# cartgr/Generating-Fair-Consensus-Statements-with-Social-Choice-on-Token-Level-MDPs

Measured on AMD Instinct MI355X. Metric: agent×candidate scorings/sec + decode steps/sec at 1/2/4/8 MI355X; % HBM roofline, higher is better.
Workload: dtype bf16

## Files before the change

### generating-fair-consensus-statements-with-social-choice-on-token-level-mdps_amd/csrc/attn.hip

```cpp
#include "cs_kernels.cuh"

#include <algorithm>
#include <vector>

namespace {

typedef __bf16 bf16x8 __attribute__((ext_vector_type(8)));
typedef __bf16 bf16x4 __attribute__((ext_vector_type(4)));
typedef float f32x4 __attribute__((ext_vector_type(4)));

constexpr int kAttnThreads = 256;
constexpr int kGroupRows = 64;
constexpr int kKeyBlock = 32;
constexpr int kMaxSplit = 32;
constexpr int kPlanMinBase = 1024;
constexpr int kMergeRows = 8;
constexpr float kLazyRescale = 8.0f;
constexpr int64_t kPlanImbalance = 4;
constexpr int kPlanTargetWgs = 512;
constexpr int kPlanMinItems = 3;

struct AttnParams {
  const __bf16* q;
  const __bf16* kp;
// ... 269 lines not shown

template <int D>
__device__ __forceinline__ void fetch_chunks(const BlockRef& r, u32x4 (&rk)[LdsTile<D>::NCH],
                                             u32x4 (&rv)[LdsTile<D>::NCH]) {
#pragma unroll
  for (int j = 0; j < LdsTile<D>::NCH; ++j) {
    const int c = static_cast<int>(threadIdx.x) + kAttnThreads * j;
    rk[j] = *reinterpret_cast<const u32x4*>(r.k + c * 8);
    rv[j] = *reinterpret_cast<const u32x4*>(r.vt + c * 8);
  }
}

template <int D>
__device__ __forceinline__ void stage_chunks(__bf16* buf, int j, const u32x4 (&rk)[LdsTile<D>::NCH],
                                             const u32x4 (&rv)[LdsTile<D>::NCH]) {
  using LT = LdsTile<D>;
  __bf16* kd = buf + (j & 1) * LT::ELEMS;
  __bf16* vd = kd + LT::KELEMS;
  const int tid = threadIdx.x;
  __bf16* kt = kd + (tid / (D / 8)) * LT::KROW + (tid % (D / 8)) * 8;
  __bf16* vt = vd + (tid >> 2) * LT::VROW + (tid & 3) * 8;
#pragma unroll
  for (int i = 0; i < LT::NCH; ++i) {
    *reinterpret_cast<u32x4*>(kt + i * (kAttnThreads / (D / 8)) * LT::KROW) = rk[i];
    *reinterpret_cast<u32x4*>(vt + i * (kAttnThreads / 4) * LT::VROW) = rv[i];
  }
}

__device__ __forceinline__ bool mine_staged(const TileRows& tr, int j) {
  return tr.active && (j % tr.kw) == tr.ks;
}

template <int D, typename Ref>
__device__ __forceinline__ void attend_staged(const AttnParams& a, const TileRows& tr, const __bf16* buf,
                                              int j, Ref ref, const bf16x8 (&qf)[D / 32],
                                              f32x4 (&o)[D / 16], float& m, float& l) {
  using LT = LdsTile<D>;
  const int col = tr.col, h4 = tr.h4;
  const __bf16* kd = buf + (j & 1) * LT::ELEMS;
  const __bf16* vd = kd + LT::KELEMS;
  KeyBlock<D> f;
#pragma unroll
  for (int ds = 0; ds < D / 32; ++ds) {
    f.k0[ds] = *reinterpret_cast<const bf16x8*>(kd + col * LT::KROW + ds * 32 + 8 * h4);
    f.k1[ds] = *reinterpret_cast<const bf16x8*>(kd + (16 + col) * LT::KROW + ds * 32 + 8 * h4);
  }
#pragma unroll
  for (int dt = 0; dt < D / 16; ++dt) {
    f.vlo[dt] = *reinterpret_cast<const bf16x4*>(vd + (dt * 16 + col) * LT::VROW + 4 * h4);
    f.vhi[dt] = *reinterpret_cast<const bf16x4*>(vd + (dt * 16 + col) * LT::VROW + 16 + 4 * h4);
  }
  attend_block<D>(a, f, ref(j).mask, qf, tr.kmin_pos, h4, o, m, l);
}

#define CS_ATTEND_STAGED(D, a, tr, lds, n_blocks, ref, qf, o, m, l)                         \
  do {                                                                                      \
    using LT_ = LdsTile<D>;                                                                 \
    const int n_ = (n_blocks);                                                              \
    __bf16* buf_ = reinterpret_cast<__bf16*>(lds);                                          \
    u32x4 rk_[LT_::NCH], rv_[LT_::NCH];                                                     \
    if (n_ > 0) {                                                                           \
      fetch_chunks<D>(ref(0), rk_, rv_);                                                    \
      stage_chunks<D>(buf_, 0, rk_, rv_);                                                   \
    }                                                                                       \
    __syncthreads();                                                                        \
    for (int j_ = 0; j_ < n_; ++j_) {                                                       \
      const bool more_ = j_ + 1 < n_;                                                       \
      if (more_) fetch_chunks<D>(ref(j_ + 1), rk_, rv_);                                    \
      if (mine_staged(tr, j_)) attend_staged<D>(a, tr, buf_, j_, ref, qf, o, m, l);   \
      if (more_) stage_chunks<D>(buf_, j_ + 1, rk_, rv_);                                   \
      __syncthreads();                                                                      \
    }                                                                                       \
  } while (0)

template <int D>
__device__ __forceinline__ void combine_waves(const TileRows& tr, char* lds, f32x4 (&o)[D / 16],
                                              float& m, float& l) {
  auto sm = reinterpret_cast<float (*)[16][LdsTile<D>::LDSW]>(lds);
  const int n_qt = tr.n_qt, kw = tr.kw, col = tr.col, h4 = tr.h4;
  l += __shfl_xor(l, 16, 64);
  l += __shfl_xor(l, 32, 64);
  if (kw > 1) {
    if (tr.active && tr.ks > 0) {
      const int sl = tr.w - n_qt;
#pragma unroll
      for (int dt = 0; dt < D / 16; ++dt)
#pragma unroll
        for (int i = 0; i < 4; ++i) sm[sl][col][dt * 16 + 4 * h4 + i] = o[dt][i];
      if (h4 == 0) {
        sm[sl][col][D] = m;
        sm[sl][col][D + 1] = l;
      }
    }
    __syncthreads();
    if (tr.active && tr.ks == 0) {
      float mt = m;
      for (int k = 1; k < kw; ++k) mt = fmaxf(mt, sm[tr.qt + n_qt * k - n_qt][col][D]);
      const float c0 = mt == -INFINITY ? 0.0f : __builtin_amdgcn_exp2f(m - mt);
      l *= c0;
#pragma unroll
      for (int dt = 0; dt < D / 16; ++dt) o[dt] *= c0;
      for (int k = 1; k < kw; ++k) {
        const int sl = tr.qt + n_qt * k - n_qt;
        const float mk = sm[sl][col][D];
        const float ck = mt == -INFINITY ? 0.0f : __builtin_amdgcn_exp2f(mk - mt);
        l = fmaf(sm[sl][col][D + 1], ck, l);
#pragma unroll
        for (int dt = 0; dt < D / 16; ++dt)
#pragma unroll
          for (int i = 0; i < 4; ++i) o[dt][i] = fmaf(sm[sl][col][dt * 16 + 4 * h4 + i], ck, o[dt][i]);
      }
      m = mt;
    }
  }
}

template <int D>
__device__ __forceinline__ void store_out(const AttnParams& a, const TileRows& tr,
                                          const f32x4 (&o)[D / 16], float l) {
  const float inv = l > 0.0f ? 1.0f / l : 0.0f;
  __bf16* orow = a.out + (tr.tok * a.H + tr.head) * D + 4 * tr.h4;
#pragma unroll
  for (int dt = 0; dt < D / 16; ++dt) {
    bf16x4 v;
#pragma unroll
    for (int i = 0; i < 4; ++i) v[i] = static_cast<__bf16>(o[dt][i] * inv);
    *reinterpret_cast<bf16x4*>(orow + dt * 16) = v;
  }
}

template <int D>
__global__ __launch_bounds__(kAttnThreads, D <= 128 ? 2 : 1)
void prefix_attn_lds_kernel(AttnParams a) {
  __shared__ __attribute__((aligned(16))) char lds[LdsTile<D>::kBytes];
  const int bid = logical_block(a.swizzle);
  const TileRows tr = tile_rows(a, bid / a.n_qg, bid % a.n_qg);
  const HistBlocks hs = hist_blocks(a, tr.hb, tr.r0, tr.r0 + tr.nrows - 1);
  const int nbp = (tr.pl + kKeyBlock - 1) / kKeyBlock;

  bf16x8 qf[D / 32];
  load_q<D>(a, tr, qf);
  f32x4 o[D / 16];
#pragma unroll
  for (int dt = 0; dt < D / 16; ++dt) o[dt] = f32x4{0.f, 0.f, 0.f, 0.f};
  float m = -INFINITY, l = 0.0f;

  const KvBase kv = kv_base(a);
  auto ref = [&](int it) {
    return it < nbp ? prefix_block<D>(a, kv, tr, it) : hist_block<D>(a, kv, tr, hs, it - nbp);
  };
  CS_ATTEND_STAGED(D, a, tr, lds, nbp + hs.n, ref, qf, o, m, l);
  combine_waves<D>(tr, lds, o, m, l);
  if (tr.vrow && tr.ks == 0) store_out<D>(a, tr, o, l);
}

#ifdef CS_TRACE_ATTN
constexpr int kAttTraceWgs = 4096;
__device__ unsigned long long g_attn_ts[kAttTraceWgs][8];
#define ATT_T(...) __VA_ARGS__
__device__ __forceinline__ void att_at(int i) {
  if (blockIdx.x < kAttTraceWgs) g_attn_ts[blockIdx.x][i] = wall_clock64();
}
#else
#define ATT_T(...)
#endif

template <int D, bool ROWS = false>
__global__ __launch_bounds__(kAttnThreads, 2)
void prefix_attn_plan_lds_kernel(AttnParams a) {
  using LT = LdsTile<D>;
  constexpr int NDS = D / 32;
  constexpr int NDT = D / 16;
  constexpr int kVImg = kKeyBlock * D * 2;
  static_assert(kAttnThreads / 64 * kVImg <= LT::kBufBytes, "the V images fit the prefix buffers");
  __shared__ __attribute__((aligned(16))) char lds[LT::kBytes];

  ATT_T(if (threadIdx.x == 0) att_at(0);)
  const int4 e = a.plan ? a.plan[blockIdx.x]
                        : int4{static_cast<int>(blockIdx.x) / a.n_qg, static_cast<int>(blockIdx.x) % a.n_qg,
                               1 << 8, 0};
  const int split = e.z & 255, n_used = e.z >> 8, slot = e.w;
  const TileRows tr = tile_rows(a, e.x, e.y);
  const int lane = tr.lane, w = tr.w, kw = tr.kw, ks = tr.ks;
  const int col = tr.col, h4 = tr.h4;
  const bool active = tr.active;

  const int nbp = (tr.pl + kKeyBlock - 1) / kKeyBlock;
  const int npi = nbp > split ? (nbp - split + n_used - 1) / n_used : 0;
  ATT_T(if (threadIdx.x == 0 && npi + tr.hb + tr.po >= 0) att_at(1);)
  const int rt0 = tr.r0 + tr.qt * 16;
  const HistBlocks hs = hist_blocks(a, tr.hb, rt0, min(rt0 + 15, tr.M - 1));
  const int n_hist = hs.n;
  const int nslot = n_used * kw;
  auto hrow_of = [&](int ih) -> int32_t {
    const int64_t sg = static_cast<int64_t>(tr.gi) * a.n_str + hs.b_lo + ih / hs.nbh;
    return a.hrow[sg * a.ldh + (ih % hs.nbh) * kKeyBlock + (lane & 31)];
  };
  int32_t hcur = 0;
  if constexpr (ROWS) {
    if (active && split * kw + ks < n_hist) hcur = hrow_of(split * kw + ks);
  }

  bf16x8 qf[NDS];
  load_q<D>(a, tr, qf);
  f32x4 o[NDT];
#pragma unroll
  for (int dt = 0; dt < NDT; ++dt) o[dt] = f32x4{0.f, 0.f, 0.f, 0.f};
  float m = -INFINITY, l = 0.0f;

  const KvBase kv = kv_base(a);
  auto ref = [&](int j) { return prefix_block<D>(a, kv, tr, split + j * n_used); };
  CS_ATTEND_STAGED(D, a, tr, lds, npi, ref, qf, o, m, l);

  ATT_T(if (threadIdx.x == 0) att_at(2);)
  if constexpr (!ROWS) {
    if (active) {
      for (int ih = split * kw + ks; ih < n_hist; ih += nslot) {
        KeyBlock<D> f;
        const BlockRef r = hist_block<D>(a, kv, tr, hs, ih);
        load_block<D>(f, r, col, h4);
        attend_block<D>(a, f, r.mask, qf, tr.kmin_pos, h4, o, m, l);
      }
    }
  } else {
    unsigned char* vimg = reinterpret_cast<unsigned char*>(lds) + w * kVImg;
    constexpr int CPK = D / 8;
    constexpr int KPI = 64 / CPK;
    const int kq = 4 * h4 + ((lane & 15) >> 2);
    const uint32_t tr_base = static_cast<uint32_t>(kq * 2 * D + 8 * (lane & 3));
    const int s2 = vimg_swz<D>(kq) >> 1;
    const int dkey = lane / CPK, dch = lane % CPK;
    typedef __attribute__((address_space(3))) bf16x4* lds_b4_ptr;
    if (active && split * kw + ks < n_hist) {
#pragma unroll
      for (int i = 0; i < kVImg / 1024; ++i)
        *reinterpret_cast<u32x4*>(vimg + 1024 * i + 16 * lane) = u32x4{0u, 0u, 0u, 0u};
    }
    if (active) {
      for (int ih = split * kw + ks; ih < n_hist; ih += nslot) {
        const BlockMask mk = hist_block<D>(a, kv, tr, hs, ih).mask;
        const int kb = mk.kb;
        const int nvalid = min(kKeyBlock, hs.hlim - kb);
        const int n_instr = (nvalid + KPI - 1) / KPI;
        auto row_ptr = [&](const __bf16* base, int64_t srow, int key) {
          return base + ((srow * a.Hkv + tr.g) * a.ldh + kb + key) * D;
        };
        const int64_t rk0 = __shfl(hcur, col, 64), rk1 = __shfl(hcur, 16 + col, 64);
        KeyBlock<D> f;
        const __bf16* kp0 = row_ptr(a.kh, rk0, col) + 8 * h4;
        const __bf16* kp1 = row_ptr(a.kh, rk1, 16 + col) + 8 * h4;
#pragma unroll
        for (int ds = 0; ds < NDS; ++ds) {
          f.k0[ds] = *reinterpret_cast<const bf16x8*>(kp0 + ds * 32);
          f.k1[ds] = *reinterpret_cast<const bf16x8*>(kp1 + ds * 32);
        }
        __builtin_amdgcn_sched_barrier(0);
        asm volatile("s_waitcnt lgkmcnt(0)" ::: "memory");
#pragma unroll 1
        for (int i = 0; i < n_instr; ++i) {
          const int k = i * KPI + dkey;
          const int64_t rv = __shfl(hcur, k, 64);
          const __bf16* vsrc = row_ptr(a.vth, rv, k) + 8 * (dch ^ vimg_swz<D>(k));
          __builtin_amdgcn_global_load_lds(vsrc, (__attribute__((address_space(3))) void*)(vimg + 1024 * i),
                                           16, 0, 0);
        }
        __builtin_amdgcn_sched_barrier(0);
        const int ihn = ih + nslot < n_hist ? ih + nslot : ih;
        const int32_t hnext = hrow_of(ihn);
        __builtin_amdgcn_sched_barrier(0);
        asm volatile("s_waitcnt vmcnt(0)" ::: "memory");
#pragma unroll
        for (int dt = 0; dt < NDT; ++dt) {
          const uint32_t o2 = tr_base + 32 * (((dt & 7) ^ s2) + (dt & ~7));
          f.vlo[dt] = __builtin_amdgcn_ds_read_tr16_b64_v4bf16((lds_b4_ptr)(vimg + o2));
          f.vhi[dt] = __builtin_amdgcn_ds_read_tr16_b64_v4bf16((lds_b4_ptr)(vimg + o2 + 32 * D));
        }
        attend_block<D>(a, f, mk, qf, tr.kmin_pos, h4, o, m, l);
        hcur = hnext;
      }
    }
    __syncthreads();
  }
  ATT_T(if (threadIdx.x == 0 && l >= 0.0f) att_at(3);)
  combine_waves<D>(tr, lds, o, m, l);
  if (!tr.vrow || ks != 0) return;
  if (n_used == 1) {
    store_out<D>(a, tr, o, l);
  } else {
    float* pr = a.part + (static_cast<int64_t>(slot) * kGroupRows + tr.qt * 16 + col) * LT::LDSW;
#pragma unroll
    for (int dt = 0; dt < NDT; ++dt)
      *reinterpret_cast<f32x4*>(pr + dt * 16 + 4 * h4) = o[dt];
    if (h4 == 0) {
      pr[D] = m;
      pr[D + 1] = l;
    }
  }
  ATT_T(if (threadIdx.x == 0) { __builtin_amdgcn_s_waitcnt(0); att_at(4); })
}

#undef CS_ATTEND_STAGED

template <int D>
__global__ __launch_bounds__(kAttnThreads) void attn_merge_kernel(AttnParams a) {
  constexpr int LDSW = D + 2;
  constexpr int NC = D / 4;
// ... 255 lines not shown
  for (int32_t gi = 0; gi < n_groups; ++gi) {
    const int32_t p = group_prefix ? group_prefix[gi] : gi;
    if (p < 0 || p >= n_prefix || prefix_len[p] < 0)
      return fail(CS_ERR_INVALID, "cs_prefix_attention_plan: group_prefix / prefix_len out of range");
    const int64_t nbp = (prefix_len[p] + kKeyBlock - 1) / kKeyBlock;
    for (int64_t qg = 0; qg < n_qg; ++qg) {
      const int64_t r0 = qg * kGroupRows;
      const int64_t nrows = std::min<int64_t>(kGroupRows, M - r0);
      const int64_t n_qt = (nrows + 15) / 16;
      const int64_t kw = n_qt == 1 ? 4 : (n_qt == 2 ? 2 : 1);
      int64_t items = 0;
      for (int64_t q = 0; q < n_qt; ++q) {
        const int64_t rt0 = r0 + 16 * q, rt1 = std::min(rt0 + 15, M - 1);
        const int64_t streams = (rt1 / rep) / T - (rt0 / rep) / T + 1;
        items = std::max(items, nbp + streams * nbh_max);
      }
      cl.push_back({gi, static_cast<int32_t>(qg), items, kw, nrows});
    }
  }
  if (base >= kPlanMinBase) {
    int64_t sum = 0, mx = 0;
    for (const Cell& c : cl) {
      sum += c.items;
      mx = std::max(mx, c.items);
    }
    if (mx * static_cast<int64_t>(cl.size()) <= kPlanImbalance * sum) return 0;
  }
  auto splits_of = [](const Cell& c, int64_t q) {
    return std::max<int64_t>(1, std::min<int64_t>(kMaxSplit, (c.items + q * c.kw - 1) / (q * c.kw)));
  };
  int64_t work = 0;
  for (const Cell& c : cl) work += (c.items + c.kw - 1) / c.kw;
  work *= Hkv;
  const int64_t q = std::max<int64_t>(kPlanMinItems, (work + kPlanTargetWgs - 1) / kPlanTargetWgs);
  std::vector<PlanCell> cells;
  cells.reserve(cl.size());
  int64_t na = 0, nm = 0, slots = 0;
  for (const Cell& c : cl) {
    const int64_t s = splits_of(c, q);
    const int64_t per = (c.items + s * c.kw - 1) / (s * c.kw);
    cells.push_back({c.gi, c.qg, static_cast<int32_t>(s), static_cast<int32_t>(per)});
    na += s * Hkv;
    if (s > 1) {
      slots += s * Hkv;
      nm += (c.nrows + kMergeRows - 1) / kMergeRows * Hkv;
    }
  }
  if (nm == 0) return 0;
  if (na + nm > 0x7fffffffLL) return fail(CS_ERR_INVALID, "cs_prefix_attention_plan: plan too large");
  if (n_attn) *n_attn = static_cast<int32_t>(na);
  if (n_merge) *n_merge = static_cast<int32_t>(nm);
  if (workspace_bytes) *workspace_bytes = static_cast<size_t>(slots) * kGroupRows * (D + 2) * sizeof(float);
  const int64_t total = na + nm;
  if (!plan) return total;
  if (plan_cap < total) return fail(CS_ERR_INVALID, "cs_prefix_attention_plan: plan_cap too small");
  std::stable_sort(cells.begin(), cells.end(),
                   [](const PlanCell& x, const PlanCell& y) { return x.per_wg > y.per_wg; });
  int32_t* pa = plan;
  int32_t* pm = plan + 4 * na;
  int32_t slot = 0;
  for (const PlanCell& c : cells) {
    const int64_t r0 = static_cast<int64_t>(c.qg) * kGroupRows;
    const int64_t nrows = std::min<int64_t>(kGroupRows, M - r0);
    for (int32_t g = 0; g < Hkv; ++g) {
      const int32_t pg = c.gi * Hkv + g;
      for (int32_t sp = 0; sp < c.splits; ++sp) {
        pa[0] = pg;
        pa[1] = c.qg;
        pa[2] = sp | (c.splits << 8);
        pa[3] = c.splits > 1 ? slot + sp : 0;
        pa += 4;
      }
      if (c.splits > 1) {
        for (int32_t ch = 0; ch < (nrows + kMergeRows - 1) / kMergeRows; ++ch) {
          pm[0] = pg;
          pm[1] = c.qg;
          pm[2] = slot;
          pm[3] = ch | (c.splits << 8);
          pm += 4;
        }
        slot += c.splits;
      }
    }
  }
  return total;
}

}

namespace {
int prefix_attention_impl(const char* name, const void* q, const void* k_prefix, const void* vt_prefix,
                          int64_t ld_prefix, const int64_t* prefix_off, const int32_t* prefix_len,
                          int32_t max_prefix_len, const int32_t* group_prefix, int32_t n_groups,
                          const void* k_hist, const void* vt_hist, const int32_t* hist_rows,
                          int64_t ld_hist, const int32_t* hist_base, int32_t n_str, int32_t T,
                          int32_t H, int32_t Hkv, int32_t D, float scale, float softcap,
                          int32_t window, const void* plan, int32_t n_attn, int32_t n_merge,
                          void* out, void* workspace, size_t workspace_bytes, cs_stream_t stream) {
  const std::string nm(name);
  if (n_groups < 0 || n_str < 0 || T < 0) return fail(CS_ERR_INVALID, nm + ": negative size");
  if (n_groups == 0 || n_str == 0 || T == 0) return CS_OK;
  if (Hkv <= 0 || H <= 0 || H % Hkv != 0 || H / Hkv > 64)
    return fail(CS_ERR_INVALID, nm + ": H must be a multiple of Hkv (<= 64 per group)");
  if (D != 64 && D != 128 && D != 256)
    return fail(CS_ERR_INVALID, nm + ": head_dim must be 64, 128 or 256");
  if (ld_prefix <= 0 || ld_prefix % kKeyBlock != 0 || ld_hist <= 0 || ld_hist % kKeyBlock != 0)
    return fail(CS_ERR_INVALID, nm + ": ld_prefix / ld_hist must be positive multiples of 32");
  if (max_prefix_len < 0 || max_prefix_len > ld_prefix)
    return fail(CS_ERR_INVALID, nm + ": max_prefix_len outside [0, ld_prefix]");
  if (!q || !k_prefix || !vt_prefix || !prefix_off || !prefix_len || !k_hist || !vt_hist ||
      !hist_base || !out || (hist_rows == nullptr) != (nm == "cs_prefix_attention"))
    return fail(CS_ERR_INVALID, nm + ": NULL pointer");
  if (!(scale > 0.0f) || softcap < 0.0f) return fail(CS_ERR_INVALID, nm + ": bad scale / softcap");
  if (plan && (n_attn <= 0 || n_merge <= 0))
    return fail(CS_ERR_INVALID, nm + ": a plan needs n_attn > 0 and n_merge > 0");
  if (plan && !workspace)
    return fail(CS_ERR_WORKSPACE, nm + ": a plan needs the workspace cs_prefix_attention_plan() sized");
  const int64_t M = static_cast<int64_t>(n_str) * T * (H / Hkv);
  const int64_t n_qg = (M + kGroupRows - 1) / kGroupRows;
  const int64_t base = static_cast<int64_t>(n_groups) * Hkv * n_qg;
  if (n_qg > 0x7fffffff || base > 0x7fffffffLL) return fail(CS_ERR_INVALID, nm + ": too many query rows");
  AttnParams a;
  a.q = static_cast<const __bf16*>(q);
  a.kp = static_cast<const __bf16*>(k_prefix);
  a.vtp = static_cast<const __bf16*>(vt_prefix);
  a.poff = prefix_off;
  a.plen = prefix_len;
  a.gpfx = group_prefix;
  a.kh = static_cast<const __bf16*>(k_hist);
  a.vth = static_cast<const __bf16*>(vt_hist);
  a.hist_base = hist_base;
  a.hrow = hist_rows;
  a.out = static_cast<__bf16*>(out);
  a.part = static_cast<float*>(workspace);
  a.plan = static_cast<const int4*>(plan);
  a.ldp = ld_prefix;
  a.ldh = ld_hist;
  a.n_grp = n_groups;
  a.n_str = n_str;
  a.T = T;
  a.H = H;
  a.Hkv = Hkv;
  a.rep = H / Hkv;
  a.n_qg = static_cast<int32_t>(n_qg);
  a.n_attn = plan ? n_attn : 0;
  a.scale = scale;
  a.softcap = softcap;
  a.inv_softcap = softcap > 0.0f ? 1.0f / softcap : 0.0f;
  a.window = window > 0 ? window : 0;
  (void)workspace_bytes;
  const int64_t nwg = plan ? n_attn : base;
  a.swizzle = (!plan && nwg % 8 == 0 && nwg >= 64) ? 1 : 0;
  hipStream_t st = static_cast<hipStream_t>(stream);
  const dim3 grid(static_cast<uint32_t>(nwg));
  const dim3 merge_grid(static_cast<uint32_t>(plan ? n_merge : 0));
#define CS_ATTN_LAUNCH(DV)                                                              \
  do {                                                                                  \
    if (hist_rows)                                                                      \
      hipLaunchKernelGGL((prefix_attn_plan_lds_kernel<DV, true>), grid, dim3(kAttnThreads), 0, st, a); \
    else if (plan)                                                                      \
      hipLaunchKernelGGL(prefix_attn_plan_lds_kernel<DV>, grid, dim3(kAttnThreads), 0, st, a); \
    else                                                                                \
      hipLaunchKernelGGL(prefix_attn_lds_kernel<DV>, grid, dim3(kAttnThreads), 0, st, a); \
    if (plan)                                                                           \
      hipLaunchKernelGGL(attn_merge_kernel<DV>, merge_grid, dim3(kAttnThreads), 0, st, a); \
  } while (0)
  if (D == 64) {
    CS_ATTN_LAUNCH(64);
  } else if (D == 128) {
    CS_ATTN_LAUNCH(128);
  } else {
    CS_ATTN_LAUNCH(256);
  }
#undef CS_ATTN_LAUNCH
  return check_launch(name);
}
}

extern "C" {

int cs_prefix_attention(const void* q, const void* k_prefix, const void* vt_prefix,
                        int64_t ld_prefix, const int64_t* prefix_off, const int32_t* prefix_len,
                        int32_t max_prefix_len, const int32_t* group_prefix, int32_t n_groups,
                        const void* k_hist, const void* vt_hist, int64_t ld_hist,
                        const int32_t* hist_base, int32_t n_str, int32_t T, int32_t H, int32_t Hkv,
                        int32_t D, float scale, float softcap, int32_t window, const void* plan,
                        int32_t n_attn, int32_t n_merge, void* out, void* workspace,
                        size_t workspace_bytes, cs_stream_t stream) {
  return prefix_attention_impl("cs_prefix_attention", q, k_prefix, vt_prefix, ld_prefix, prefix_off,
                               prefix_len, max_prefix_len, group_prefix, n_groups, k_hist, vt_hist,
                               nullptr, ld_hist, hist_base, n_str, T, H, Hkv, D, scale, softcap,
                               window, plan, n_attn, n_merge, out, workspace, workspace_bytes, stream);
}

int cs_prefix_attention_rows(const void* q, const void* k_prefix, const void* vt_prefix,
                             int64_t ld_prefix, const int64_t* prefix_off, const int32_t* prefix_len,
                             int32_t max_prefix_len, const int32_t* group_prefix, int32_t n_groups,
                             const void* k_hist, const void* v_hist, const int32_t* hist_rows,
                             int64_t ld_hist, const int32_t* hist_base, int32_t n_str, int32_t T,
                             int32_t H, int32_t Hkv, int32_t D, float scale, float softcap,
                             int32_t window, const void* plan, int32_t n_attn, int32_t n_merge,
                             void* out, void* workspace, size_t workspace_bytes, cs_stream_t stream) {
  if (!hist_rows) return fail(CS_ERR_INVALID, "cs_prefix_attention_rows: NULL hist_rows");
  return prefix_attention_impl("cs_prefix_attention_rows", q, k_prefix, vt_prefix, ld_prefix,
                               prefix_off, prefix_len, max_prefix_len, group_prefix, n_groups,
                               k_hist, v_hist, hist_rows, ld_hist, hist_base, n_str, T, H, Hkv, D,
                               scale, softcap, window, plan, n_attn, n_merge, out, workspace,
                               workspace_bytes, stream);
}

#ifdef CS_TRACE_ATTN
int cs_attn_trace_read(unsigned long long* out) {
  (void)hipMemcpyFromSymbol(out, HIP_SYMBOL(g_attn_ts), sizeof(g_attn_ts));
  static unsigned long long zero[kAttTraceWgs][8];
  (void)hipMemcpyToSymbol(HIP_SYMBOL(g_attn_ts), zero, sizeof(zero));
  return 0;
}
#endif

int cs_hist_rows_update(const int32_t* src_rows, int32_t* dst_rows, const int64_t* parent,
                        const int32_t* hist_base, int64_t S, int32_t ld_hist, int64_t row_base,
                        int64_t n_rows, cs_stream_t stream) {
  if (S < 0 || ld_hist <= 0 || row_base < 0) return fail(CS_ERR_INVALID, "cs_hist_rows_update: bad shape");
  if (row_base + S > n_rows)
    return fail(CS_ERR_INVALID, "cs_hist_rows_update: rows row_base .. row_base + S - 1 exceed the buffer's n_rows");
  if (S == 0) return CS_OK;
  if (!src_rows || !dst_rows || !parent || !hist_base)
    return fail(CS_ERR_INVALID, "cs_hist_rows_update: NULL pointer");
  if (src_rows == dst_rows) return fail(CS_ERR_INVALID, "cs_hist_rows_update: source and destination must differ");
  if (S > 0x7fffffffLL || row_base + S > 0x7fffffffLL || (S * ld_hist + 255) / 256 > 0x7fffffffLL)
    return fail(CS_ERR_INVALID, "cs_hist_rows_update: table too large");
  hipLaunchKernelGGL(hist_rows_kernel, dim3(static_cast<uint32_t>((S * ld_hist + 255) / 256)), dim3(256), 0,
                     static_cast<hipStream_t>(stream), src_rows, dst_rows, parent, hist_base, S, ld_hist,
                     row_base);
  return check_launch("cs_hist_rows_update");
}

}

namespace {
int rope_place_impl(const void* qkv, int64_t ld_qkv, const float* part, int32_t splits,
                    const float* inv_freq, const int32_t* prefix_len, const int32_t* group_prefix,
                    int32_t n_groups, const int32_t* hist_base, int32_t n_str, int32_t T, int32_t H,
                    int32_t Hkv, int32_t D, void* q_out, void* k_hist, void* vt_hist,
                    int64_t ld_hist, int32_t v_rows, cs_stream_t stream) {
  if (n_groups < 0 || n_str < 0 || T < 0) return fail(CS_ERR_INVALID, "cs_rope_place: negative size");
  if (n_groups == 0 || n_str == 0 || T == 0) return CS_OK;
  if (H <= 0 || Hkv <= 0 || D <= 0 || D % 2 != 0 || ld_qkv < static_cast<int64_t>(H + 2 * Hkv) * D)
    return fail(CS_ERR_INVALID, "cs_rope_place: bad head layout");
  if (ld_hist < T) return fail(CS_ERR_INVALID, "cs_rope_place: ld_hist < T");
  if (!inv_freq || !prefix_len || !hist_base || !q_out || !k_hist || !vt_hist)
    return fail(CS_ERR_INVALID, "cs_rope_place: NULL pointer");
  RopeParams r;
  r.qkv = static_cast<const __bf16*>(qkv);
  r.ldqkv = ld_qkv;
  r.part = part;
  r.splits = splits;
  r.inv_freq = inv_freq;
  r.plen = prefix_len;
  r.gpfx = group_prefix;
  r.hist_base = hist_base;
  r.q_out = static_cast<__bf16*>(q_out);
  r.kh = static_cast<__bf16*>(k_hist);
  r.vth = static_cast<__bf16*>(vt_hist);
  r.ldh = ld_hist;
  r.v_rows = v_rows;
  r.n_tok = static_cast<int64_t>(n_groups) * n_str * T;
  r.n_str = n_str;
  r.T = T;
  r.H = H;
  r.Hkv = Hkv;
  r.D = D;
  if (D % 8 != 0 || D > 256) return fail(CS_ERR_INVALID, "cs_rope_place: head_dim must be a multiple of 8, <= 256");
  if (r.n_tok > 0x7fffffffLL) return fail(CS_ERR_INVALID, "cs_rope_place: too many tokens");
  const int64_t n_tiles = ld_hist / 32;
  const int64_t n_vwg = static_cast<int64_t>(n_groups) * n_str * Hkv * n_tiles;
  r.skip_v = (!part && !v_rows && T >= 32 && ld_hist % 32 == 0 && ld_qkv % 8 == 0 &&
              reinterpret_cast<uintptr_t>(qkv) % 16 == 0 && n_vwg <= 0x7fffffffLL) ? 1 : 0;
  const bool p8 = part ? true
                       : (ld_qkv % 8 == 0 && reinterpret_cast<uintptr_t>(qkv) % 16 == 0 && D % 16 == 0);
  const int64_t n_items = static_cast<int64_t>(H + 2 * Hkv) * (D / 2) / (p8 ? 8 : 4);
  const int64_t n_split = (n_items + kRopeItems - 1) / kRopeItems;
  if (r.n_tok * n_split > 0x7fffffffLL) return fail(CS_ERR_INVALID, "cs_rope_place: too many tokens");
  const dim3 grid(static_cast<uint32_t>(r.n_tok * n_split));
  if (part && splits <= 2)
    hipLaunchKernelGGL((rope_place_kernel<8, true, 2>), grid, dim3(256), 0, static_cast<hipStream_t>(stream),
                       r, static_cast<int32_t>(n_split));
  else if (part && splits <= 4)
    hipLaunchKernelGGL((rope_place_kernel<8, true, 4>), grid, dim3(256), 0, static_cast<hipStream_t>(stream),
                       r, static_cast<int32_t>(n_split));
  else if (part)
    hipLaunchKernelGGL((rope_place_kernel<8, true, 8>), grid, dim3(256), 0, static_cast<hipStream_t>(stream),
                       r, static_cast<int32_t>(n_split));
  else if (p8)
    hipLaunchKernelGGL(rope_place_kernel<8>, grid, dim3(256), 0, static_cast<hipStream_t>(stream), r,
                       static_cast<int32_t>(n_split));
  else
    hipLaunchKernelGGL(rope_place_kernel<4>, grid, dim3(256), 0, static_cast<hipStream_t>(stream), r,
                       static_cast<int32_t>(n_split));
  if (r.skip_v)
    hipLaunchKernelGGL(v_tile_place_kernel, dim3(static_cast<uint32_t>(n_vwg)), dim3(256), 0,
                       static_cast<hipStream_t>(stream), r, static_cast<int32_t>(n_tiles));
  return check_launch("cs_rope_place");
}

int rope_place_splitk_impl(const char* name, const float* part, int32_t splits, const float* inv_freq,
// ... 224 lines not shown
```

Baseline: 563.3.

## Add wide 32x32 MFMA attention kernel for unplanned D=128 prefill

Adds a new attention kernel for head dimension 128 that uses 32x32x16 bf16 MFMA tiles, 64-key blocks, register-prefetched double-buffered LDS staging with XOR swizzles, and lazy softmax rescaling. Each wave owns 32 query rows, and the output goes through an LDS image so global stores are coalesced. The kernel is dispatched when no split plan, no history rows, no softcap and no window apply. The aim is higher MFMA throughput and fewer LDS round trips per key block, at the cost of a large, specialised code path with higher register pressure.

Measured after the change: 572.9, median of 6. 1.02x the previous value.

```diff
diff --git a/generating-fair-consensus-statements-with-social-choice-on-token-level-mdps_amd/csrc/attn.hip b/generating-fair-consensus-statements-with-social-choice-on-token-level-mdps_amd/csrc/attn.hip
--- a/generating-fair-consensus-statements-with-social-choice-on-token-level-mdps_amd/csrc/attn.hip
+++ b/generating-fair-consensus-statements-with-social-choice-on-token-level-mdps_amd/csrc/attn.hip
@@ -445,6 +445,329 @@
   CS_ATTEND_STAGED(D, a, tr, lds, nbp + hs.n, ref, qf, o, m, l);
   combine_waves<D>(tr, lds, o, m, l);
   if (tr.vrow && tr.ks == 0) store_out<D>(a, tr, o, l);
+}
+
+typedef float f32x16 __attribute__((ext_vector_type(16)));
+
+constexpr int kWideWaves = 4;
+constexpr int kWideBlock = 64;
+
+template <int D, int NW>
+struct WideLds {
+  static_assert(D == 128, "the chunk swizzles below are written for 256-byte K rows");
+  static constexpr int NT = 64 * NW;
+  static constexpr int KBYTES = kWideBlock * D * 2;
+  static constexpr int VTILE = D * 64;
+  static constexpr int BUF = KBYTES + 2 * VTILE;
+  static constexpr int NCH = kWideBlock * (D / 8) / NT;
+  static constexpr int QIMG = 32 * D * 2;
+  static_assert(NW * QIMG <= 2 * BUF, "every wave's row image fits the two key buffers");
+  static_assert(NCH >= 2 && NCH % 2 == 0, "a thread's chunks split evenly over the two tiles");
+};
+
+template <int NW>
+__device__ __forceinline__ TileRows wide_rows(const AttnParams& a, int pg, int qg) {
+  TileRows r;
+  r.gi = pg / a.Hkv;
+  r.g = pg % a.Hkv;
+  const int p = a.gpfx ? a.gpfx[r.gi] : r.gi;
+  r.M = a.n_str * a.T * a.rep;
+  r.r0 = qg * 32 * NW;
+  r.nrows = min(32 * NW, r.M - r.r0);
+  r.n_qt = (r.nrows + 31) >> 5;
+  r.kw = 1;
+  const int tid = threadIdx.x;
+  r.w = tid >> 6;
+  r.lane = tid & 63;
+  r.qt = r.w;
+  r.ks = 0;
+  r.active = r.w < r.n_qt;
+  r.col = r.lane & 31;
+  r.h4 = r.lane >> 5;
+  const int row = r.r0 + r.w * 32 + r.col;
+  r.vrow = row < r.M;
+  const int rr = r.vrow ? row : r.M - 1;
+  const int jh = rr % a.rep, bt = rr / a.rep;
+  r.t = bt % a.T;
+  r.b = bt / a.T;
+  r.tok = (static_cast<int64_t>(r.gi) * a.n_str + r.b) * a.T + r.t;
+  r.head = r.g * a.rep + jh;
+  r.hb = *a.hist_base;
+  r.pl = a.plen[p];
+  r.po = a.poff[p];
+  r.hv = min(r.hb + r.t + 1, static_cast<int>(a.ldh));
+  r.kmin_pos = INT32_MIN;
+  return r;
+}
+
+struct WideRef {
+  const __bf16 *k0, *vt0, *k1, *vt1;
+  int kb, bb;
+};
+
+template <int D, int NW>
+__device__ __forceinline__ void wide_fetch(const WideRef& r, u32x4 (&rk)[WideLds<D, NW>::NCH],
+                                           u32x4 (&rv)[WideLds<D, NW>::NCH]) {
+  using WL = WideLds<D, NW>;
+  const int tid = threadIdx.x;
+#pragma unroll
+  for (int j = 0; j < WL::NCH; ++j) {
+    const bool first = j < WL::NCH / 2;
+    const int c = tid + WL::NT * (j % (WL::NCH / 2));
+    rk[j] = *reinterpret_cast<const u32x4*>((first ? r.k0 : r.k1) + c * 8);
+    rv[j] = *reinterpret_cast<const u32x4*>((first ? r.vt0 : r.vt1) + c * 8);
+  }
+}
+
+template <int D, int NW>
+__device__ __forceinline__ void wide_stage(char* buf, const u32x4 (&rk)[WideLds<D, NW>::NCH],
+                                           const u32x4 (&rv)[WideLds<D, NW>::NCH]) {
+  using WL = WideLds<D, NW>;
+  typedef uint32_t u32x2 __attribute__((ext_vector_type(2)));
+  const int tid = threadIdx.x;
+#pragma unroll
+  for (int j = 0; j < WL::NCH; ++j) {
+    const int half = j < WL::NCH / 2 ? 0 : 1;
+    const int c = tid + WL::NT * (j % (WL::NCH / 2));
+    const int krow = c >> 4, kch = c & 15;
+    *reinterpret_cast<u32x4*>(buf + (half * 32 + krow) * 256 + ((kch ^ (krow & 15)) << 4)) = rk[j];
+    const int d = c >> 2, s = (c >> 1) & 1, u = c & 1, g = (d >> 2) & 3;
+    char* vrow = buf + WL::KBYTES + half * WL::VTILE + d * 64 + u * 8;
+    *reinterpret_cast<u32x2*>(vrow + (((2 * s) ^ g) << 4)) = u32x2{rv[j][0], rv[j][1]};
+    *reinterpret_cast<u32x2*>(vrow + (((2 * s + 1) ^ g) << 4)) = u32x2{rv[j][2], rv[j][3]};
+  }
+}
+
+template <int D, int NW>
+__global__ __launch_bounds__(64 * NW, 2)
+void prefix_attn_wide_kernel(AttnParams a) {
+  using WL = WideLds<D, NW>;
+  constexpr int NDS = D / 16;
+  constexpr int NDT = D / 32;
+  __shared__ __attribute__((aligned(16))) char lds[2 * WL::BUF];
+  const int bid = logical_block(a.swizzle);
+  const TileRows tr = wide_rows<NW>(a, bid / a.n_qg, bid % a.n_qg);
+  const int row1 = tr.r0 + tr.nrows - 1;
+  const HistBlocks hs = hist_blocks(a, tr.hb, tr.r0, row1);
+  const int nbp = (tr.pl + kWideBlock - 1) / kWideBlock;
+  const int n_st = hs.n / hs.nbh;
+  const int hlim_last = min(tr.hb + (row1 / a.rep) % a.T + 1, static_cast<int>(a.ldh));
+  const int nbh_full = (hs.hlim + kWideBlock - 1) / kWideBlock;
+  const int nbh_last = (hlim_last + kWideBlock - 1) / kWideBlock;
+  const int n = nbp + (n_st - 1) * nbh_full + nbh_last;
+  const int r = tr.col, h = tr.h4;
+
+  const int w = __builtin_amdgcn_readfirstlane(tr.w);
+  const int wr0 = tr.r0 + 32 * w, wr1 = min(wr0 + 31, tr.M - 1);
+  const bool wact = wr0 < tr.M;
+  const int wb_lo = (wr0 / a.rep) / a.T, wb_hi = (wr1 / a.rep) / a.T, wt_hi = (wr1 / a.rep) % a.T;
+
+  const KvBase kv = kv_base(a);
+  struct Cursor {
+    int it, si, j, kb;
+    int64_t off;
+  };
+  const int64_t hoff0 = ((static_cast<int64_t>(tr.gi) * a.n_str + hs.b_lo) * a.Hkv + tr.g) * a.ldh * D;
+  const int64_t hstride = static_cast<int64_t>(a.Hkv) * a.ldh * D;
+  const Cursor c0 = {0, 0, 0, 0, nbp > 0 ? (static_cast<int64_t>(tr.g) * a.ldp + tr.po) * D : hoff0};
+  auto step = [&](Cursor& c) {
+    ++c.it;
+    if (c.it < nbp || (c.it > nbp && ++c.j < (c.si == n_st - 1 ? nbh_last : nbh_full))) {
+      c.kb += kWideBlock;
+      c.off += kWideBlock * D;
+    } else {
+      if (c.it > nbp) ++c.si;
+      c.j = 0;
+      c.kb = 0;
+      c.off = hoff0 + c.si * hstride;
+    }
+  };
+  auto ref = [&](const Cursor& c) {
+    WideRef x;
+    const bool hist = c.it >= nbp;
+    const int lim = hist ? (c.si == n_st - 1 ? hlim_last : hs.hlim) : tr.pl;
+    x.k0 = (hist ? kv.kh : kv.kp) + c.off;
+    x.vt0 = (hist ? kv.vth : kv.vtp) + c.off;
+    const bool two = c.kb + kKeyBlock < lim;
+    x.k1 = two ? x.k0 + kKeyBlock * D : x.k0;
+    x.vt1 = two ? x.vt0 + kKeyBlock * D : x.vt0;
+    x.kb = c.kb;
+    x.bb = hist ? hs.b_lo + c.si : -1;
+    return x;
+  };
+
+  bf16x8 qf[NDS];
+  {
+    const __bf16* qrow = a.q + (tr.tok * a.H + tr.head) * D + 8 * h;
+#pragma unroll
+    for (int ds = 0; ds < NDS; ++ds) {
+      if (tr.vrow) {
+        qf[ds] = *reinterpret_cast<const bf16x8*>(qrow + ds * 16);
+      } else {
+#pragma unroll
+        for (int e = 0; e < 8; ++e) qf[ds][e] = static_cast<__bf16>(0.0f);
+      }
+    }
+  }
+  f32x16 o[NDT];
+#pragma unroll
+  for (int dt = 0; dt < NDT; ++dt)
+#pragma unroll
+    for (int i = 0; i < 16; ++i) o[dt][i] = 0.0f;
+  float m = -INFINITY, l = 0.0f;
+  const float sl2 = a.scale * kLog2e;
+
+  const int kx = h ^ (r & 15);
+  const int vx = h ^ ((r >> 2) & 3);
+  const int koff = r * 256;
+  const int voff0 = WL::KBYTES + r * 64 + (vx << 4), voff1 = WL::KBYTES + r * 64 + ((vx ^ 2) << 4);
+
+  u32x4 rk[WL::NCH], rv[WL::NCH];
+  Cursor ca = c0, cf = c0;
+  wide_fetch<D, NW>(ref(cf), rk, rv);
+  wide_stage<D, NW>(lds, rk, rv);
+  step(cf);
+  if (n > 1) {
+    wide_fetch<D, NW>(ref(cf), rk, rv);
+    step(cf);
+  }
+  for (int j = 0; j < n; ++j) {
+    __syncthreads();
+    if (j + 1 < n) wide_stage<D, NW>(lds + ((j + 1) & 1) * WL::BUF, rk, rv);
+    const WideRef x = ref(ca);
+    step(ca);
+    const BlockMask mk = block_mask(tr, x.kb, x.bb >= 0, x.bb);
+    bool mine = wact;
+    if (x.bb >= 0) {
+      const int wl = (x.bb < wb_lo || x.bb > wb_hi)
+                         ? 0 : min(tr.hb + (x.bb == wb_hi ? wt_hi : a.T - 1) + 1, static_cast<int>(a.ldh));
+      mine = mine && mk.kb < wl;
+    }
+    const char* buf = lds + (j & 1) * WL::BUF;
+    f32x16 s0, s1;
+    if (mine) {
+#pragma unroll
+      for (int i = 0; i < 16; ++i) s0[i] = s1[i] = 0.0f;
+      bf16x8 kf[NDS / 2][4];
+      auto read_k = [&](int g) {
+#pragma unroll
+        for (int e = 0; e < 2; ++e) {
+          const char* kp = buf + koff + ((kx ^ (2 * (2 * g + e))) << 4);
+          kf[g][2 * e] = *reinterpret_cast<const bf16x8*>(kp);
+          kf[g][2 * e + 1] = *reinterpret_cast<const bf16x8*>(kp + 32 * 256);
+        }
+      };
+      read_k(0);
+      read_k(1);
+      __builtin_amdgcn_sched_barrier(0);
+#pragma unroll
+      for (int g = 0; g < NDS / 2; ++g) {
+        if (g + 2 < NDS / 2) read_k(g + 2);
+#pragma unroll
+        for (int e = 0; e < 2; ++e) {
+          s0 = __builtin_amdgcn_mfma_f32_32x32x16_bf16(kf[g][2 * e], qf[2 * g + e], s0, 0, 0, 0);
+          s1 = __builtin_amdgcn_mfma_f32_32x32x16_bf16(kf[g][2 * e + 1], qf[2 * g + e], s1, 0, 0, 0);
+        }
+        __builtin_amdgcn_sched_barrier(0);
+      }
+    }
+    if (j + 2 < n) {
+      wide_fetch<D, NW>(ref(cf), rk, rv);
+      step(cf);
+    }
+    if (mine) {
+      bf16x8 vf[4][NDT];
+      auto read_v = [&](int g) {
+#pragma unroll
+        for (int dt = 0; dt < NDT; ++dt)
+          vf[g][dt] = *reinterpret_cast<const bf16x8*>(buf + ((g & 1) ? voff1 : voff0) + (g >> 1) * WL::VTILE +
+                                                       dt * 32 * 64);
+      };
+      const int jhi = mk.lim - mk.kb - 4 * h;
+      if (__ballot(mk.lim - mk.kb < kWideBlock) != 0) {
+#pragma unroll
+        for (int i = 0; i < 16; ++i) {
+          const int ki = (i & 3) + 8 * (i >> 2);
+          s0[i] = ki < jhi ? s0[i] : -INFINITY;
+          s1[i] = 32 + ki < jhi ? s1[i] : -INFINITY;
+        }
+      }
+      auto mx = [](float x, float y) { return __builtin_amdgcn_fmed3f(x, y, INFINITY); };
+      float b0 = mx(s0[0], s1[0]), b1 = mx(s0[1], s1[1]);
+#pragma unroll
+      for (int i = 2; i < 16; i += 2) {
+        b0 = mx(b0, mx(s0[i], s1[i]));
+        b1 = mx(b1, mx(s0[i + 1], s1[i + 1]));
+      }
+      float bm = mx(b0, b1);
+      bm *= sl2;
+      {
+        const auto sw = __builtin_amdgcn_permlane32_swap(__float_as_uint(bm), __float_as_uint(bm), false, false);
+        bm = fmaxf(__uint_as_float(sw[0]), __uint_as_float(sw[1]));
+      }
+      float mn = m;
+      if (__ballot(bm > m + kLazyRescale) != 0) {
+        mn = fmaxf(m, bm);
+        const float alpha = mn == -INFINITY ? 1.0f : __builtin_amdgcn_exp2f(m - mn);
+        l *= alpha;
+#pragma unroll
+        for (int dt = 0; dt < NDT; ++dt)
+#pragma unroll
+          for (int i = 0; i < 16; ++i) o[dt][i] *= alpha;
+      }
+      m = mn;
+      const float ms = mn == -INFINITY ? 0.0f : mn;
+      float ps = 0.0f;
+      bf16x8 pb[2][2];
+#pragma unroll
+      for (int i = 0; i < 16; ++i) {
+        const float p0 = __builtin_amdgcn_exp2f(fmaf(s0[i], sl2, -ms));
+        const float p1 = __builtin_amdgcn_exp2f(fmaf(s1[i], sl2, -ms));
+        ps += p0 + p1;
+        pb[0][i >> 3][i & 7] = static_cast<__bf16>(p0);
+        pb[1][i >> 3][i & 7] = static_cast<__bf16>(p1);
+      }
+      l += ps;
+      read_v(0);
+      read_v(1);
+      __builtin_amdgcn_sched_barrier(0);
+#pragma unroll
+      for (int g = 0; g < 4; ++g) {
+        if (g + 2 < 4) read_v(g + 2);
+#pragma unroll
+        for (int dt = 0; dt < NDT; ++dt)
+          o[dt] = __builtin_amdgcn_mfma_f32_32x32x16_bf16(vf[g][dt], pb[g >> 1][g & 1], o[dt], 0, 0, 0);
+        __builtin_amdgcn_sched_barrier(0);
+      }
+    }
+  }
+  l += __shfl_xor(l, 32, 64);
+  const float inv = l > 0.0f ? 1.0f / l : 0.0f;
+  __syncthreads();
+  {
+    char* img = lds + w * WL::QIMG;
+#pragma unroll
+    for (int dt = 0; dt < NDT; ++dt)
+#pragma unroll
+      for (int g = 0; g < 4; ++g) {
+        bf16x4 v;
+#pragma unroll
+        for (int i = 0; i < 4; ++i) v[i] = static_cast<__bf16>(o[dt][4 * g + i] * inv);
+        *reinterpret_cast<bf16x4*>(img + r * 256 + (((4 * dt + g) ^ (r & 15)) << 4) + 8 * h) = v;
+      }
+    __builtin_amdgcn_fence(__ATOMIC_RELEASE, "wavefront");
+    __builtin_amdgcn_wave_barrier();
+    __builtin_amdgcn_fence(__ATOMIC_ACQUIRE, "wavefront");
+    const int64_t mine_off = tr.vrow ? (tr.tok * a.H + tr.head) * D : -1;
+    const int lr = tr.lane >> 4, ch = tr.lane & 15;
+#pragma unroll
+    for (int i = 0; i < 8; ++i) {
+      const int row = 4 * i + lr;
+      const int64_t off = __shfl(mine_off, row, 64);
+      const u32x4 v = *reinterpret_cast<const u32x4*>(img + row * 256 + ((ch ^ (row & 15)) << 4));
+      if (off >= 0) *reinterpret_cast<u32x4*>(a.out + off + ch * 8) = v;
+    }
+  }
 }
 
 #ifdef CS_TRACE_ATTN
@@ -1006,6 +1329,16 @@
   const int64_t nwg = plan ? n_attn : base;
   a.swizzle = (!plan && nwg % 8 == 0 && nwg >= 64) ? 1 : 0;
   hipStream_t st = static_cast<hipStream_t>(stream);
+  if (!plan && !hist_rows && D == 128 && softcap == 0.0f && a.window == 0 && 32 % a.rep == 0 && T >= 32) {
+    constexpr int kRows = 32 * kWideWaves;
+    const int64_t n_wg = (M + kRows - 1) / kRows;
+    const int64_t nw = static_cast<int64_t>(n_groups) * Hkv * n_wg;
+    a.n_qg = static_cast<int32_t>(n_wg);
+    a.swizzle = (nw % 8 == 0 && nw >= 64) ? 1 : 0;
+    hipLaunchKernelGGL((prefix_attn_wide_kernel<128, kWideWaves>), dim3(static_cast<uint32_t>(nw)),
+                       dim3(64 * kWideWaves), 0, st, a);
+    return check_launch(name);
+  }
   const dim3 grid(static_cast<uint32_t>(nwg));
   const dim3 merge_grid(static_cast<uint32_t>(plan ? n_merge : 0));
 #define CS_ATTN_LAUNCH(DV)                                                              \
```
